# YiKwanwoo2/mycelium-fea-project

Measured on AMD Instinct MI355X. Metric: DOF solved/sec + CG iters to 1e-8; SpMV achieved HBM GB/s vs roofline, higher is better.
Workload: dtype f64 (CG; f32 AMG V-cycle); 1 GPU; C3_1M: 6x8 tiles, 1062000 DOF, 1008054 free DOF, 364342 elements, load step 20/40; n_dof=1062000, n_free_dof=1008054, n_elems=364342, precond=gamg, parallelism=1gpu, cg_kernel=lanes, n_lanes=353600

## Files before the change

mycelium-fea-project_amd/csrc/amg.hip:

```cpp
#include "amg_dev.hpp"

namespace mfea {

__device__ __forceinline__ int64_t setup_block(int x1, int64_t nmain = -1) {
  if (!x1) return nmain < 0 ? xcd_block() : xcd_block_n(nmain);
  return (blockIdx.x & 7) ? -1 : (int64_t)(blockIdx.x >> 3);
}


template <int ND>
__device__ __forceinline__ double dinv_row(const AmgLevD& L, int64_t i) {
  const AmgMatD& A = L.A;
  double g = 0.0;
  if (i - (threadIdx.x & 63) < A.rg.hi) {
    int64_t base;
    int w;
    slice_of(A, i, base, w);
    if (i >= A.rg.lo && i < A.rg.hi) {
      double D[ND * ND], Di[ND * ND];
      bload<ND>(A.val32, A.npos, base, D);
      binv<ND>(D, Di);
#pragma unroll
      for (int c = 0; c < ND * ND; ++c) L.dinv32[i * (ND * ND) + c] = (float)Di[c];
      double rs[ND];
// ... 1232 lines not shown
#pragma unroll
      for (int a = 0; a < 3; ++a) v.x[3 * row + a] = xk[a];
    } else {
      v.x[3 * row] = 0.0;
      v.x[3 * row + 1] = c == 3 ? 0.0 : (c == 2 ? dy_bot : dy_top);
      v.x[3 * row + 2] = 0.0;
    }
  }
  if (!block_publish<2>(acc, partials, ticket, red_out)) return;
  for (int64_t k = threadIdx.x; k < nzero; k += kBlock) zero[k] = 0.0;
  if (threadIdx.x == 0) cg_state_init(st, red_out[0], red_out[1], rtol, atol, norm, max_it, reg);
}

template <int BS, class F>
__device__ __forceinline__ void tile_rows(int64_t n, F&& f) {
  const int lane = threadIdx.x & 63;
  const int64_t nt = (n + 2 * BS - 1) / (2 * BS);
  for (int64_t tile = xcd_block(); tile < nt; tile += gridDim.x)
#pragma unroll
    for (int m = 0; m < 2; ++m) {
      const int64_t i = tile * (2 * BS) + m * BS + threadIdx.x;
      if (i - lane < n) f(i);
    }
}

template <int ND, bool FIRST, int BS, bool DIST, int KW = 1, bool TILE = false>
__global__ __launch_bounds__(BS) void k_amg_cg_w(int j, AmgLevD L0, AmgCg cg, Slot* slots, double* part,
                                                 AmgDist d) {
  double acc[4] = {0.0, 0.0, 0.0, 0.0};
  const int64_t stride = (int64_t)gridDim.x * BS;
  const int lane = threadIdx.x & 63;
  auto row = [&](int64_t i) {
    const int64_t ii = i < cg.hi ? i : cg.hi - 1;
    int64_t base;
    int w;
    slice_of(L0.A, ii, base, w);
    double y[ND], u[ND], r[ND];
    vload<ND>(cg.u, ii, u);
    vload<ND>(cg.r, ii, r);
#pragma unroll
    for (int a = 0; a < ND; ++a) y[a] = 0.0;
    sell_mac<ND, false, KW, true>(L0.A.col, L0.A.sym, L0.A.npos, base, w, cg.u, y);
    if (i < cg.lo || i >= cg.hi) return;
    if constexpr (DIST) {
      for (int t = d.gptr[i]; t < d.gptr[i + 1]; ++t) {
        const int64_t q = d.gslot[t];
        double s6[6], m[ND * ND], ug[ND];
#pragma unroll
        for (int c = 0; c < 6; ++c) s6[c] = d.sval[(int64_t)c * d.G + q];
        sym_to<ND>(s6, m);
        vload<ND>(d.urecv, d.grecv[t], ug);
#pragma unroll
        for (int a = 0; a < ND; ++a)
#pragma unroll
          for (int b = 0; b < ND; ++b) y[a] = fma(m[a * ND + b], ug[b], y[a]);
      }
    }
    vstore<ND>(cg.w, i, y);
#pragma unroll
    for (int a = 0; a < ND; ++a) {
      acc[0] = fma(r[a], u[a], acc[0]);
      acc[1] = fma(y[a], u[a], acc[1]);
      acc[2] = fma(r[a], r[a], acc[2]);
      acc[3] = fma(u[a], u[a], acc[3]);
    }
  };
  if constexpr (TILE) {
    tile_rows<BS>(cg.hi, row);
  } else {
    for (int64_t i = cg.lo64() + xcd_block() * BS + threadIdx.x; i - lane < cg.hi; i += stride) row(i);
  }
  store_block_partial<BS>(acc, part_buf(part, FIRST ? 0 : ((j & 1) ^ 1)));
  if (FIRST && blockIdx.x == 0 && threadIdx.x == 0) {
    Slot s0;
    s0.v[0] = s0.v[1] = s0.v[2] = s0.v[3] = 0.0;
    s0.alpha = s0.beta = s0.res = 0.0;
    s0.flag = kInit;
    s0.pad = 0;
    slots[0] = s0;
  }
}

template <int ND, int BS, int KW>
__global__ __launch_bounds__(BS) void k_amg_up_w(int j, int first, AmgLevD L, AmgLevD N, AmgCg cg, AmgFuseD f,
                                                 Slot* slots, double* part) {
  extern __shared__ float ul[];
  double acc[4] = {0.0, 0.0, 0.0, 0.0};
  const AmgMatD& T = L.PT;
  const int lane = threadIdx.x & 63;
  const int64_t n = cg.hi;
  const int64_t nt = (n + 2 * BS - 1) / (2 * BS);
  const float* src = N.coarsest ? N.x : N.e;
  for (int64_t tile = xcd_block(); tile < nt; tile += gridDim.x) {
    const int64_t r0 = tile * (2 * BS);
#pragma unroll
    for (int m = 0; m < 2; ++m) {
      const int64_t a = r0 + m * BS + threadIdx.x;
      if (a - lane >= n) continue;
      const int64_t aa = a < n ? a : n - 1;
      int64_t base;
      int w;
      slice_of(T, aa, base, w);
      const int64_t i = L.pt_row[aa];
      float y[ND];
      vload<ND>(L.t, i, y);
      sell_mac<ND, false, 3>(T.col, T.val32, T.npos, base, w, src, y);
      if (a < n) {
        vstore<ND>(cg.u, i, y);
        vstore<ND>(ul, i - r0, y);
      }
    }
    const int h0 = f.hptr[tile], h1 = f.hptr[tile + 1];
    for (int h = h0 + (int)threadIdx.x; h < h1; h += BS) {
      const int64_t a = f.hpt[h], i = f.hrow[h];
      const int sa = T.sptr[a >> 6], sb = T.sptr[(a >> 6) + 1];
      const int64_t base = (int64_t)sa * 64 + (a & 63);
      float y[ND];
      vload<ND>(L.t, i, y);
      sell_mac<ND, false, 3>(T.col, T.val32, T.npos, base, sb - sa, src, y);
      vstore<ND>(ul, 2 * BS + (h - h0), y);
    }
    __syncthreads();
#pragma unroll
    for (int m = 0; m < 2; ++m) {
      const int64_t i = r0 + m * BS + threadIdx.x;
      if (i - lane >= n) continue;
      const int64_t ii = i < n ? i : n - 1;
      int64_t base;
      int w;
      slice_of(L.A, ii, base, w);
      double y[ND], u[ND], r[ND];
      vload<ND>(ul, ii - r0, u);
      vload<ND>(cg.r, ii, r);
#pragma unroll
      for (int a = 0; a < ND; ++a) y[a] = 0.0;
      sell_mac<ND, false, KW, true>(f.lcol, L.A.sym, L.A.npos, base, w, (const float*)ul, y);
      if (i >= n) continue;
      vstore<ND>(cg.w, i, y);
#pragma unroll
      for (int a = 0; a < ND; ++a) {
        acc[0] = fma(r[a], u[a], acc[0]);
        acc[1] = fma(y[a], u[a], acc[1]);
        acc[2] = fma(r[a], r[a], acc[2]);
        acc[3] = fma(u[a], u[a], acc[3]);
      }
    }
    if (tile + gridDim.x < nt) __syncthreads();
  }
  store_block_partial<BS>(acc, part_buf(part, first ? 0 : ((j & 1) ^ 1)));
  if (first && blockIdx.x == 0 && threadIdx.x == 0) {
    Slot s0;
    s0.v[0] = s0.v[1] = s0.v[2] = s0.v[3] = 0.0;
    s0.alpha = s0.beta = s0.res = 0.0;
    s0.flag = kInit;
    s0.pad = 0;
    slots[0] = s0;
  }
}

struct PxLive {
  double alpha[kAmgPxSlots], beta[kAmgPxSlots];
  int64_t off[kAmgPxSlots];
  int n;
};
__device__ __forceinline__ void px_records(const Slot* __restrict__ slots, const AmgPx& px, PxLive& L) {
  if (threadIdx.x < 64) {
    const int t = threadIdx.x, k = px.k0 + t;
    bool run = false;
    double a = 0.0, b = 0.0;
    if (t < px.cnt) {
      const Slot& rec = slots[k + 1];
      run = rec.flag == kRun && rec.pad == 0;
      a = rec.alpha;
      b = rec.beta;
    }
    const unsigned long long m = __ballot(run);
    if (run) {
      const int q = __popcll(m & ((1ull << t) - 1ull));
      L.alpha[q] = a;
      L.beta[q] = b;
      L.off[q] = (int64_t)amg_px_slot(k) * px.stride;
    }
    if (t == 0) L.n = __popcll(m);
  }
  __syncthreads();
}
template <int ND>
__device__ __forceinline__ void px_row(const AmgCg& cg, const AmgPx& px, const PxLive& L, int64_t i) {
  const int n = L.n;
  if (n == 0) return;
  double p[ND], x[ND];
  vload<ND>(cg.p, i, p);
  vload<ND>(cg.x, i, x);
#pragma unroll 4
  for (int t = 0; t < n; ++t) {
    double u[ND];
    vload<ND>(px.uh + L.off[t], i, u);
    const double alpha = L.alpha[t], beta = L.beta[t];
#pragma unroll
    for (int a = 0; a < ND; ++a) {
      p[a] = fma(beta, p[a], u[a]);
      x[a] = fma(alpha, p[a], x[a]);
    }
  }
  vstore<ND>(cg.p, i, p);
  vstore<ND>(cg.x, i, x);
}
template <int ND>
__global__ __launch_bounds__(kCgBS) void k_amg_px_replay(AmgCg cg, const Slot* slots, AmgPx px) {
  __shared__ PxLive live;
  px_records(slots, px, live);
  const int64_t stride = (int64_t)gridDim.x * kCgBS;
  for (int64_t i = cg.lo + (int64_t)blockIdx.x * kCgBS + threadIdx.x; i < cg.hi; i += stride)
    px_row<ND>(cg, px, live, i);
}

template <int ND, int BS, bool REPLAY = false, bool TILE = false>
__global__ __launch_bounds__(BS) void k_amg_rnorm(AmgCg cg, double* cpart, const Slot* slots, AmgPx px) {
  __shared__ PxLive live;
  if constexpr (REPLAY) px_records(slots, px, live);
  double acc[4] = {0.0, 0.0, 0.0, 0.0};
  const int64_t stride = (int64_t)gridDim.x * BS;
  const int lane = threadIdx.x & 63;
  auto row = [&](int64_t i) {
    if (i < cg.lo || i >= cg.hi) return;
    double r[ND];
    vload<ND>(cg.r, i, r);
    if constexpr (REPLAY) px_row<ND>(cg, px, live, i);
#pragma unroll
    for (int a = 0; a < ND; ++a) acc[2] = fma(r[a], r[a], acc[2]);
  };
  if constexpr (TILE) {
// ... 523 lines not shown

void launch_amg_row0_inverse(hipStream_t s, const AmgCg& cg, int32_t* inv, int64_t n_rows) {
  (void)hipMemsetAsync(inv, 0xff, (size_t)n_rows * sizeof(int32_t), s);
  if (cg.hi <= cg.lo) return;
  hipLaunchKernelGGL(k_amg_row0_inverse, rows_grid(cg.hi - cg.lo), dim3(kBlock), 0, s, cg, inv);
}

void launch_amg_start(hipStream_t s, int nd, const SellOp& op, const uint8_t* code, double dy_top, double dy_bot,
                      const CgVecs& v, double* partials, unsigned* ticket, double* red_out, const AmgLevD& L0,
                      const AmgCg& cg, const int32_t* inv, double rtol, double atol, int norm, int max_it,
                      double reg, SolveState* st, double* zero, int64_t nzero, const BcForm& bc) {
  const dim3 grid((unsigned)grid_rows(op.N > 0 ? op.N : 1));
  with_bc(bc, [&](auto g, auto ld) {
    using GM = decltype(g);
    using LD = decltype(ld);
    if (nd == 2)
      hipLaunchKernelGGL((k_amg_start<2, GM, LD>), grid, dim3(kBlock), 0, s, op, code, dy_top, dy_bot, v, partials,
                         ticket, red_out, L0, cg, inv, rtol, atol, norm, max_it, reg, st, zero, nzero, g, ld);
    else
      hipLaunchKernelGGL((k_amg_start<3, GM, LD>), grid, dim3(kBlock), 0, s, op, code, dy_top, dy_bot, v, partials,
                         ticket, red_out, L0, cg, inv, rtol, atol, norm, max_it, reg, st, zero, nzero, g, ld);
  });
}

template <int ND, int BS>
static void w_bs(hipStream_t s, int j, bool first, const AmgLevD& L0, const AmgCg& cg, Slot* slots,
                 double* part, const AmgDist* d) {
  const dim3 g((unsigned)amg_w_grid(cg));
  const AmgDist dd = d ? *d : AmgDist{};
  if (d) {
    if (first) hipLaunchKernelGGL((k_amg_cg_w<ND, true, BS, true>), g, dim3(BS), 0, s, j, L0, cg, slots, part, dd);
    else hipLaunchKernelGGL((k_amg_cg_w<ND, false, BS, true>), g, dim3(BS), 0, s, j, L0, cg, slots, part, dd);
  } else if (cg.w_k == 2) {
    if (first) hipLaunchKernelGGL((k_amg_cg_w<ND, true, BS, false, 2>), g, dim3(BS), 0, s, j, L0, cg, slots, part, dd);
    else hipLaunchKernelGGL((k_amg_cg_w<ND, false, BS, false, 2>), g, dim3(BS), 0, s, j, L0, cg, slots, part, dd);
  } else {
    if (first) hipLaunchKernelGGL((k_amg_cg_w<ND, true, BS, false>), g, dim3(BS), 0, s, j, L0, cg, slots, part, dd);
    else hipLaunchKernelGGL((k_amg_cg_w<ND, false, BS, false>), g, dim3(BS), 0, s, j, L0, cg, slots, part, dd);
  }
}
template <int ND, int BS>
static void w_tile_bs(hipStream_t s, int j, bool first, const AmgLevD& L0, const AmgCg& cg, Slot* slots,
                      double* part) {
  const dim3 g((unsigned)amg_w_grid(cg));
  const AmgDist dd{};
  if (cg.w_k == 2) {
    if (first) hipLaunchKernelGGL((k_amg_cg_w<ND, true, BS, false, 2, true>), g, dim3(BS), 0, s, j, L0, cg, slots, part, dd);
    else hipLaunchKernelGGL((k_amg_cg_w<ND, false, BS, false, 2, true>), g, dim3(BS), 0, s, j, L0, cg, slots, part, dd);
  } else {
    if (first) hipLaunchKernelGGL((k_amg_cg_w<ND, true, BS, false, 1, true>), g, dim3(BS), 0, s, j, L0, cg, slots, part, dd);
    else hipLaunchKernelGGL((k_amg_cg_w<ND, false, BS, false, 1, true>), g, dim3(BS), 0, s, j, L0, cg, slots, part, dd);
  }
}
template <int ND>
static void w_nd(hipStream_t s, int j, bool first, const AmgLevD& L0, const AmgCg& cg, Slot* slots,
                 double* part, const AmgDist* d) {
  if (w_tiled(cg) && !d) {
    if (cg.w_tile == 1408) w_tile_bs<ND, 704>(s, j, first, L0, cg, slots, part);
    else w_tile_bs<ND, 512>(s, j, first, L0, cg, slots, part);
    return;
  }
  switch (amg_w_block(cg)) {
    case 512: w_bs<ND, 512>(s, j, first, L0, cg, slots, part, d); break;
    case 576: w_bs<ND, 576>(s, j, first, L0, cg, slots, part, d); break;
    case 640: w_bs<ND, 640>(s, j, first, L0, cg, slots, part, d); break;
    case 704: w_bs<ND, 704>(s, j, first, L0, cg, slots, part, d); break;
    case 768: w_bs<ND, 768>(s, j, first, L0, cg, slots, part, d); break;
    case 1024: w_bs<ND, 1024>(s, j, first, L0, cg, slots, part, d); break;
    default: w_bs<ND, kCgBS>(s, j, first, L0, cg, slots, part, d); break;
  }
}
void launch_amg_cg_w(hipStream_t s, int nd, int j, bool first, const AmgLevD& L0, const AmgCg& cg,
                     Slot* slots, double* part, const AmgDist* d) {
  if (nd == 2) w_nd<2>(s, j, first, L0, cg, slots, part, d);
  else w_nd<3>(s, j, first, L0, cg, slots, part, d);
}

template <int ND, int BS>
static void up_w_bs(hipStream_t s, int j, bool first, const AmgLevD& L0, const AmgLevD& L1, const AmgCg& cg,
                    const AmgFuseD& f, Slot* slots, double* part) {
  const dim3 g((unsigned)amg_w_grid(cg));
  const size_t lds = (size_t)(2 * BS + f.hcap) * ND * sizeof(float);
  const int fi = first ? 1 : 0;
  if (cg.w_k == 2) hipLaunchKernelGGL((k_amg_up_w<ND, BS, 2>), g, dim3(BS), lds, s, j, fi, L0, L1, cg, f, slots, part);
  else hipLaunchKernelGGL((k_amg_up_w<ND, BS, 1>), g, dim3(BS), lds, s, j, fi, L0, L1, cg, f, slots, part);
}
void launch_amg_up_w(hipStream_t s, int nd, int j, bool first, const AmgLevD& L0, const AmgLevD& L1,
                     const AmgCg& cg, const AmgFuseD& f, Slot* slots, double* part) {
  if (cg.w_tile == 1408) {
    if (nd == 2) up_w_bs<2, 704>(s, j, first, L0, L1, cg, f, slots, part);
    else up_w_bs<3, 704>(s, j, first, L0, L1, cg, f, slots, part);
  } else {
    if (nd == 2) up_w_bs<2, 512>(s, j, first, L0, L1, cg, f, slots, part);
    else up_w_bs<3, 512>(s, j, first, L0, L1, cg, f, slots, part);
  }
}

template <int ND, bool REPLAY>
static void rnorm_nd(hipStream_t s, const AmgCg& cg, double* cpart, const Slot* slots, const AmgPx& px) {
  const dim3 g((unsigned)amg_w_grid(cg));
  if (w_tiled(cg)) {
    if (cg.w_tile == 1408) hipLaunchKernelGGL((k_amg_rnorm<ND, 704, REPLAY, true>), g, dim3(704), 0, s, cg, cpart, slots, px);
    else hipLaunchKernelGGL((k_amg_rnorm<ND, 512, REPLAY, true>), g, dim3(512), 0, s, cg, cpart, slots, px);
    return;
  }
  switch (amg_w_block(cg)) {
    case 512: hipLaunchKernelGGL((k_amg_rnorm<ND, 512, REPLAY>), g, dim3(512), 0, s, cg, cpart, slots, px); break;
    case 576: hipLaunchKernelGGL((k_amg_rnorm<ND, 576, REPLAY>), g, dim3(576), 0, s, cg, cpart, slots, px); break;
    case 640: hipLaunchKernelGGL((k_amg_rnorm<ND, 640, REPLAY>), g, dim3(640), 0, s, cg, cpart, slots, px); break;
    case 704: hipLaunchKernelGGL((k_amg_rnorm<ND, 704, REPLAY>), g, dim3(704), 0, s, cg, cpart, slots, px); break;
    case 768: hipLaunchKernelGGL((k_amg_rnorm<ND, 768, REPLAY>), g, dim3(768), 0, s, cg, cpart, slots, px); break;
    case 1024: hipLaunchKernelGGL((k_amg_rnorm<ND, 1024, REPLAY>), g, dim3(1024), 0, s, cg, cpart, slots, px); break;
    default: hipLaunchKernelGGL((k_amg_rnorm<ND, kCgBS, REPLAY>), g, dim3(kCgBS), 0, s, cg, cpart, slots, px); break;
  }
}
void launch_amg_rnorm(hipStream_t s, int nd, const AmgCg& cg, double* cpart) {
  if (nd == 2) rnorm_nd<2, false>(s, cg, cpart, nullptr, AmgPx{});
  else rnorm_nd<3, false>(s, cg, cpart, nullptr, AmgPx{});
}
void launch_amg_rnorm_px(hipStream_t s, int nd, const AmgCg& cg, double* cpart, const Slot* slots,
                         const AmgPx& px) {
  if (nd == 2) rnorm_nd<2, true>(s, cg, cpart, slots, px);
  else rnorm_nd<3, true>(s, cg, cpart, slots, px);
}
void launch_amg_px_replay(hipStream_t s, int nd, const AmgCg& cg, const Slot* slots, const AmgPx& px) {
  if (cg.hi <= cg.lo) return;
  int64_t g = (cg.hi - cg.lo + kCgBS - 1) / kCgBS;
  g = g > kCgMaxG ? kCgMaxG : g;
  if (nd == 2) hipLaunchKernelGGL(k_amg_px_replay<2>, dim3((unsigned)g), dim3(kCgBS), 0, s, cg, slots, px);
  else hipLaunchKernelGGL(k_amg_px_replay<3>, dim3((unsigned)g), dim3(kCgBS), 0, s, cg, slots, px);
}

void launch_amg_gsum(hipStream_t s, const AmgCg& cg, const double* part_q, const AmgDist& d, int q) {
  double* all = d.gall[q];
  const int r = d.rank, zw = d.zero_w;
  switch (pu_of_grid(amg_w_grid(cg))) {
    case 1: hipLaunchKernelGGL(k_amg_gsum<1>, dim3(1), dim3(64), 0, s, part_q, all, r, zw, d.gsend); break;
    case 2: hipLaunchKernelGGL(k_amg_gsum<2>, dim3(1), dim3(64), 0, s, part_q, all, r, zw, d.gsend); break;
    case 4: hipLaunchKernelGGL(k_amg_gsum<4>, dim3(1), dim3(64), 0, s, part_q, all, r, zw, d.gsend); break;
    default: hipLaunchKernelGGL(k_amg_gsum<8>, dim3(1), dim3(64), 0, s, part_q, all, r, zw, d.gsend); break;
  }
}

void launch_amg_pack_u(hipStream_t s, int nd, const AmgCg& cg, const AmgDist& d) {
  if (d.n_send <= 0) return;
  if (nd == 2) hipLaunchKernelGGL(k_amg_pack_u<2>, rows_grid(d.n_send), dim3(kBlock), 0, s, cg, d);
  else hipLaunchKernelGGL(k_amg_pack_u<3>, rows_grid(d.n_send), dim3(kBlock), 0, s, cg, d);
}

template <int ND, int BS, bool DIST, bool LAZY = false>
static void upd_bs(hipStream_t s, int j, const AmgLevD& L0, const AmgCg& cg, Slot* slots,
                   SolveState* st, double* part, const AmgDist& d) {
  const int64_t gw = amg_w_grid(cg);
  int64_t gu = (cg.hi - cg.lo + BS - 1) / BS;
  gu = gu < 1 ? 1 : (gu > kCgMaxG ? kCgMaxG : gu);
  const dim3 g((unsigned)gu);
  switch (DIST ? 1 : pu_of_grid(gw)) {
    case 1: hipLaunchKernelGGL((k_amg_cg_update<ND, 1, BS, DIST, LAZY>), g, dim3(BS), 0, s, j, L0, cg, slots, st, part, d); break;
    case 2: hipLaunchKernelGGL((k_amg_cg_update<ND, 2, BS, DIST, LAZY>), g, dim3(BS), 0, s, j, L0, cg, slots, st, part, d); break;
    case 4: hipLaunchKernelGGL((k_amg_cg_update<ND, 4, BS, DIST, LAZY>), g, dim3(BS), 0, s, j, L0, cg, slots, st, part, d); break;
    default: hipLaunchKernelGGL((k_amg_cg_update<ND, 8, BS, DIST, LAZY>), g, dim3(BS), 0, s, j, L0, cg, slots, st, part, d); break;
  }
}
template <int ND>
static void upd_nd(hipStream_t s, int j, const AmgLevD& L0, const AmgCg& cg, Slot* slots,
                   SolveState* st, double* part, const AmgDist* d, bool lazy) {
  if (d) upd_bs<ND, kCgBS, true>(s, j, L0, cg, slots, st, part, *d);
  else if (lazy) upd_bs<ND, kCgBS, false, true>(s, j, L0, cg, slots, st, part, AmgDist{});
// ... 114 lines not shown
```

mycelium-fea-project_amd/csrc/amg_dev.hpp:

```cpp
#pragma once
#include "amg_kernels.hpp"
#include "device_util.hpp"

namespace mfea {

template <int ND, class T, class C>
__device__ __forceinline__ void bload(const T* __restrict__ v, int64_t , int64_t q, C* m) {
#pragma unroll
  for (int c = 0; c < ND * ND; ++c) m[c] = (C)v[q * (ND * ND) + c];
}
template <int ND, class T, class C>
__device__ __forceinline__ void bstore(T* __restrict__ v, int64_t , int64_t q, const C* m) {
#pragma unroll
  for (int c = 0; c < ND * ND; ++c) v[q * (ND * ND) + c] = (T)m[c];
}
template <int ND>
constexpr int nsym() { return ND * (ND + 1) / 2; }
template <int ND, class T, class C>
__device__ __forceinline__ void bload_sym(const T* __restrict__ v, int64_t , int64_t q, C* m) {
  constexpr int NS = nsym<ND>();
  C t[NS];
#pragma unroll
  for (int c = 0; c < NS; ++c) t[c] = (C)v[q * NS + c];
  if constexpr (ND == 2) {
// ... 133 lines not shown
  return slot_wave(M, t0, t1, q, row, k, xcd_block());
}

__device__ __forceinline__ int32_t uniform_load(const int32_t* p, int64_t i) {
  return ((const __attribute__((address_space(4))) int32_t*)p)[i];
}
__device__ __forceinline__ void slice_of(const AmgMatD& M, int64_t row, int64_t& base, int& width) {
  const int s = __builtin_amdgcn_readfirstlane((int)(row >> 6));
  const int a = uniform_load(M.sptr, s), b = uniform_load(M.sptr, s + 1);
  base = (int64_t)a * 64 + (row & 63);
  width = b - a;
}

template <int ND>
constexpr int mac_unroll() { return ND == 2 ? 4 : 2; }

template <int ND, int U, int S, bool SUB, bool SYM, class TV, class XP, class C, class CI>
__device__ __forceinline__ void sell_step(const CI* __restrict__ col, const TV* __restrict__ val,
                                          int64_t base, int k, int ws, int sub, XP x, C* y) {
  int32_t c[U];
  int64_t q[U];
  C m[U][ND * ND], xc[U][ND];
#pragma unroll
  for (int u = 0; u < U; ++u) {
    q[u] = k + u < ws ? base + (int64_t)((k + u) * S + sub) * 64 : base;
    c[u] = k + u < ws ? col[q[u]] : -1;
  }
#pragma unroll
  for (int u = 0; u < U; ++u) {
    if constexpr (SYM) bload_sym<ND>(val, 0, q[u], m[u]);
    else bload<ND>(val, 0, q[u], m[u]);
  }
#pragma unroll
  for (int u = 0; u < U; ++u) vload<ND>(x, c[u] >= 0 ? c[u] : 0, xc[u]);
#pragma unroll
  for (int u = 0; u < U; ++u) {
#pragma unroll
    for (int b = 0; b < ND; ++b) {
      if constexpr (SYM) xc[u][b] = keep_or_zero(xc[u][b], c[u] >= 0);
      else xc[u][b] = c[u] >= 0 ? xc[u][b] : (C)0;
    }
#pragma unroll
    for (int a = 0; a < ND; ++a)
#pragma unroll
      for (int b = 0; b < ND; ++b)
        y[a] = fma(SUB ? -m[u][a * ND + b] : m[u][a * ND + b], xc[u][b], y[a]);
  }
}
template <int ND, int UMAX, int S, bool SUB, bool SYM, class TV, class XP, class C, class CI>
__device__ __forceinline__ int sell_step_by(const CI* __restrict__ col, const TV* __restrict__ val,
                                            int64_t base, int k, int rem, int ws, int sub, XP x, C* y) {
  if (UMAX >= 16 && rem > 8) {
    sell_step<ND, (UMAX >= 16 ? 16 : 1), S, SUB, SYM>(col, val, base, k, ws, sub, x, y);
    return 16;
  }
  if (UMAX >= 8 && rem > 4) {
    sell_step<ND, (UMAX >= 8 ? 8 : 1), S, SUB, SYM>(col, val, base, k, ws, sub, x, y);
    return 8;
  }
  if (UMAX >= 4 && rem > 2) {
    sell_step<ND, (UMAX >= 4 ? 4 : 1), S, SUB, SYM>(col, val, base, k, ws, sub, x, y);
    return 4;
  }
  if (rem > 1) {
    sell_step<ND, 2, S, SUB, SYM>(col, val, base, k, ws, sub, x, y);
    return 2;
  }
  sell_step<ND, 1, S, SUB, SYM>(col, val, base, k, ws, sub, x, y);
  return 1;
}
template <int ND, int UMAX, int S, bool SUB, bool SYM, class TV, class XP, class C, class CI>
__device__ __forceinline__ void sell_steps(const CI* __restrict__ col, const TV* __restrict__ val,
                                           int64_t base, int wu, int ws, int sub, XP x, C* y) {
  for (int k = 0; k < wu;) k += sell_step_by<ND, UMAX, S, SUB, SYM>(col, val, base, k, wu - k, ws, sub, x, y);
}
template <int ND, bool SUB, int K = 2, bool SYM = false, class TV, class XP, class C, class CI>
__device__ __forceinline__ void sell_mac(const CI* __restrict__ col, const TV* __restrict__ val,
                                         int64_t , int64_t base, int w,
                                         XP x, C* y) {
  constexpr int UMAX = mac_unroll<ND>() << (K - 1);
  sell_steps<ND, UMAX, 1, SUB, SYM>(col, val, base, w, w, 0, x, y);
}

template <int ND, class TD, class C>
__device__ __forceinline__ void dinv_load(const TD* __restrict__ dinv, int64_t i, C* Di) {
#pragma unroll
  for (int c = 0; c < ND * ND; ++c) Di[c] = (C)dinv[i * (ND * ND) + c];
}
template <int ND, class C>
__device__ __forceinline__ void dinv_mul(const C* Di, C s, const C* v, C* o) {
#pragma unroll
  for (int a = 0; a < ND; ++a) {
    C acc = 0;
#pragma unroll
    for (int b = 0; b < ND; ++b) acc = fma(Di[a * ND + b], v[b], acc);
    o[a] = s * acc;
  }
}
template <int ND, class TD, class C>
__device__ __forceinline__ void dinv_apply(const TD* __restrict__ dinv, int64_t , int64_t i, C s,
                                           const C* v, C* o) {
  C Di[ND * ND];
  dinv_load<ND>(dinv, i, Di);
  dinv_mul<ND>(Di, s, v, o);
}

template <int ND, bool TX, int U, class TX_, class TY_>
__device__ __forceinline__ void pair_sum_u(int t0, int t1, const int32_t* __restrict__ la,
                                           const int32_t* __restrict__ lb, const TX_* __restrict__ X,
                                           const TY_* __restrict__ Y, double* C) {
  for (int t = t0; t < t1; t += U) {
    int32_t ia[U], ib[U];
#pragma unroll
    for (int u = 0; u < U; ++u) {
      const int tt = t + u < t1 ? t + u : t0;
      ia[u] = la[tt];
      ib[u] = lb[tt];
    }
    double x[U][ND * ND], y[U][ND * ND];
#pragma unroll
    for (int u = 0; u < U; ++u) {
      bload<ND>(X, 0, ia[u], x[u]);
      bload<ND>(Y, 0, ib[u], y[u]);
    }
#pragma unroll
    for (int u = 0; u < U; ++u) {
#pragma unroll
      for (int c = 0; c < ND * ND; ++c) x[u][c] = keep_or_zero(x[u][c], t + u < t1);
      if (TX) mtm_acc<ND>(x[u], y[u], C);
      else mm_acc<ND>(x[u], y[u], C);
    }
  }
}
template <int ND, bool TX, class TX_, class TY_>
__device__ __forceinline__ void pair_sum(int t0, int t1, const int32_t* __restrict__ la,
                                         const int32_t* __restrict__ lb, const TX_* __restrict__ X,
                                         int64_t , const TY_* __restrict__ Y, int64_t , double* C) {
  pair_sum_u<ND, TX, 4>(t0, t1, la, lb, X, Y, C);
}
template <int ND, int U, class TX_>
__device__ __forceinline__ void list_sum_u(int t0, int t1, const int32_t* __restrict__ la,
                                           const TX_* __restrict__ X, double* S) {
  for (int t = t0; t < t1; t += U) {
    int32_t ia[U];
#pragma unroll
    for (int u = 0; u < U; ++u) ia[u] = la[t + u < t1 ? t + u : t0];
    double x[U][ND * ND];
#pragma unroll
    for (int u = 0; u < U; ++u) bload<ND>(X, 0, ia[u], x[u]);
#pragma unroll
    for (int u = 0; u < U; ++u)
#pragma unroll
      for (int c = 0; c < ND * ND; ++c) S[c] += keep_or_zero(x[u][c], t + u < t1);
  }
}
template <int ND, class TX_>
__device__ __forceinline__ void list_sum(int t0, int t1, const int32_t* __restrict__ la,
                                         const TX_* __restrict__ X, int64_t , double* S) {
  list_sum_u<ND, 4>(t0, t1, la, X, S);
}

constexpr double kRhoFloor = 2.0;
constexpr double kRhoSafety = 1.45;

__device__ __forceinline__ double amg_omega(const double* __restrict__ om) {
  return (4.0 / 3.0) / (om[0] > 0.0 ? om[0] : fmax(kRhoFloor, om[1] / kRhoSafety));
// ... 22 lines not shown
```

mycelium-fea-project_amd/csrc/amg_kernels.hpp:

```cpp
#pragma once
#include <hip/hip_runtime.h>
#include <stdint.h>

#include "kernels.hpp"

namespace mfea {

struct RowRange {
  int64_t lo = 0, hi = 0;
  int64_t p0 = 0, p1 = 0;
  int64_t pf = 0, pl = 0;
  int64_t s0 = 0, s1 = 0;
  int64_t rows() const { return hi > lo ? hi - lo : 0; }
  __host__ __device__ int64_t lo64() const { return lo & ~(int64_t)63; }
  int64_t span() const { return hi > lo ? hi - lo64() : 0; }
  int64_t npos() const { return p1 > p0 ? p1 - p0 : 0; }
};

struct AmgMatD {
  int64_t n = 0;
  int64_t npos = 0;
  int32_t wmax = 0;
  RowRange rg;
  const int32_t* sptr = nullptr;
// ... 125 lines not shown
  float* dt = nullptr;
  float* lov = nullptr;
  float* upv = nullptr;
  double* y = nullptr;
};
void launch_sweep_setup(hipStream_t s, int nd, const SweepD& sw, const AmgLevD& L0);
void launch_sweep(hipStream_t s, int nd, const SweepD& sw, const AmgCg& cg, const int32_t* gate);

struct AmgDist {
  int rank = 0;
  int zero_w = 0;
  double* gall[2] = {nullptr, nullptr};
  double* gsend = nullptr;
  const int32_t* gptr = nullptr;
  const int32_t* gslot = nullptr;
  const int32_t* grecv = nullptr;
  const double* sval = nullptr;
  int64_t G = 0;
  const int32_t* send_rows = nullptr;
  int64_t n_send = 0;
  double* usend = nullptr;
  const double* urecv = nullptr;
};

void launch_amg_a0(hipStream_t s, int nd, const AmgLevD& L0, const SellOp& sop, const int32_t* row0,
                   const int32_t* a0_ptr, const int32_t* a0_a, double reg, bool full = false);
constexpr int kSetupDinv = 1, kSetupP = 2, kSetupAP = 4, kSetupAC = 8, kSetupAll = 15;
void launch_amg_level_setup(hipStream_t s, int nd, const AmgLevD& L, const AmgLevD* next, bool level0,
                            int stage = kSetupAll);
void launch_amg_compact_setup(hipStream_t s, int nd, const AmgLevD* lev, int nlev, int coll = 0, int l0 = 0);
constexpr int kCompactPT = 1, kCompactRT = 2, kCompactAT = 4, kCompactAll = 7;
void launch_amg_compact_level(hipStream_t s, int nd, const AmgLevD* lev, int l, int parts);
void launch_amg_down(hipStream_t s, int nd, const AmgLevD& L, const AmgLevD& N);
void launch_amg_up(hipStream_t s, int nd, const AmgLevD& L, const AmgLevD& N, float* e);
bool launch_amg_setup_fused(hipStream_t s, int nd, const AmgLevD* lev, int nlev, int coll,
                            const AmgMergeD* mg = nullptr);
void launch_amg_vcycle(hipStream_t s, int nd, const AmgLevD* lev, int nlev, const AmgCg& cg,
                       int tail, const int32_t* gate, int l0 = 0, const AmgMergeD* mg = nullptr);
constexpr int kStepResid = 0, kStepRestrict = 1, kStepProlong = 2, kStepPost = 3;
void launch_amg_vstep(hipStream_t s, int nd, const AmgLevD* lev, int l, const AmgCg& cg, int step,
                      const int32_t* gate);
void launch_xpack(hipStream_t s, const void* src, const int32_t* idx, int64_t n, int width, int bytes, void* buf);
constexpr int kMaxXPairs = 48;
struct XPairs {
  int n = 0;
  int64_t off[kMaxXPairs + 1] = {};
  const void* src[kMaxXPairs] = {};
  void* dst[kMaxXPairs] = {};
  const int32_t* sidx[kMaxXPairs] = {};
  const int32_t* ridx[kMaxXPairs] = {};
};
void launch_xcopy(hipStream_t s, const XPairs& pr, int width, int bytes);
struct GallCopy {
  int n = 0;
  const double* gsend[64] = {};
  double* gall[64] = {};
  int rank[64] = {};
};
void launch_gall_copy(hipStream_t s, const GallCopy& g);
void launch_xunpack(hipStream_t s, const void* buf, const int32_t* idx, int64_t n, int width, int bytes, void* dst);
void launch_amg_xinit_rows(hipStream_t s, int nd, const AmgLevD& N, const int32_t* rows, int64_t n,
                           const int32_t* gate);
void launch_amg_bound_max(hipStream_t s, double* const* omegas, int n);
int amg_restrict_lanes(const AmgLevD& L);
int amg_op_lanes(const AmgLevD& L);
int amg_down_lanes(const AmgLevD& L);
int amg_up_lanes(const AmgLevD& L);
bool amg_compact_ok(const AmgLevD* lev, int nlev, int l0);
int amg_tail_level(const int64_t* rows, int nlev, int64_t max_rows);
void launch_amg_cg_init(hipStream_t s, int nd, const AmgLevD& L0, const AmgCg& cg, const double* b_row);
void launch_amg_cg_w(hipStream_t s, int nd, int j, bool first, const AmgLevD& L0, const AmgCg& cg,
                     Slot* slots, double* part, const AmgDist* d = nullptr);
struct AmgFuseD {
  int on = 0;
  int hcap = 0;
  const int32_t* hptr = nullptr;
  const int32_t* hrow = nullptr;
  const int32_t* hpt = nullptr;
  const int16_t* lcol = nullptr;
};
constexpr int64_t kAmgFuseLds = 48 * 1024;
inline bool amg_fuse_tile_ok(int64_t B) { return B == 1408 || B == 1024; }
inline int64_t amg_fuse_halo_cap(int nd, int64_t B) { return kAmgFuseLds / (4 * nd) - B; }
void launch_amg_up_w(hipStream_t s, int nd, int j, bool first, const AmgLevD& L0, const AmgLevD& L1,
                     const AmgCg& cg, const AmgFuseD& f, Slot* slots, double* part);
void launch_amg_row0_inverse(hipStream_t s, const AmgCg& cg, int32_t* inv, int64_t n_rows);
void launch_amg_start(hipStream_t s, int nd, const SellOp& op, const uint8_t* code, double dy_top, double dy_bot,
                      const CgVecs& v, double* partials, unsigned* ticket, double* red_out, const AmgLevD& L0,
                      const AmgCg& cg, const int32_t* inv, double rtol, double atol, int norm, int max_it,
                      double reg, SolveState* st, double* zero, int64_t nzero, const BcForm& bc);
void launch_amg_rnorm(hipStream_t s, int nd, const AmgCg& cg, double* cpart);
constexpr int kAmgPxSlots = 17;
struct AmgPx {
  const float* uh = nullptr;
  int64_t stride = 0;
  int k0 = 0;
  int cnt = 0;
};
__host__ __device__ inline int amg_px_slot(int k) { return k == 0 ? 0 : 1 + (k - 1) % (kAmgPxSlots - 1); }
void launch_amg_rnorm_px(hipStream_t s, int nd, const AmgCg& cg, double* cpart, const Slot* slots,
                         const AmgPx& px);
void launch_amg_px_replay(hipStream_t s, int nd, const AmgCg& cg, const Slot* slots, const AmgPx& px);
void launch_amg_gsum(hipStream_t s, const AmgCg& cg, const double* part_q, const AmgDist& d, int q);
void launch_amg_pack_u(hipStream_t s, int nd, const AmgCg& cg, const AmgDist& d);
void launch_amg_cg_update(hipStream_t s, int nd, int j, const AmgLevD& L0, const AmgCg& cg,
                          Slot* slots, SolveState* st, double* part,
                          const AmgDist* d = nullptr, bool lazy = false);
void launch_amg_finish(hipStream_t s, int nd, const AmgCg& cg, double* x_row);
int64_t amg_w_grid(const AmgCg& cg);

}
```

mycelium-fea-project_amd/csrc/device_util.hpp:

```cpp
#pragma once
#include <type_traits>

#include "kernels.hpp"

namespace mfea {

__device__ __forceinline__ double wave_sum(double v) {
#pragma unroll
  for (int off = 32; off > 0; off >>= 1) v += __shfl_xor(v, off, 64);
  return v;
}

template <int CTRL>
__device__ __forceinline__ double dpp_d(double v) {
  const int lo = __builtin_amdgcn_update_dpp(0, __double2loint(v), CTRL, 0xF, 0xF, false);
  const int hi = __builtin_amdgcn_update_dpp(0, __double2hiint(v), CTRL, 0xF, 0xF, false);
  return __hiloint2double(hi, lo);
}
__device__ __forceinline__ double readlane_d(double v, int lane) {
  const int lo = __builtin_amdgcn_readlane(__double2loint(v), lane);
  const int hi = __builtin_amdgcn_readlane(__double2hiint(v), lane);
  return __hiloint2double(hi, lo);
}
__device__ __forceinline__ double wave_allsum(double v) {
// ... 332 lines not shown
#pragma unroll
    for (int u = 0; u < U; ++u) {
      idx[u] = base + (int64_t)(k0 + u < len ? k0 + u : k0) * 64;
      j[u] = k0 + u < len ? op.s_col[idx[u]] : 0;
    }
    uint8_t c[U];
#pragma unroll
    for (int u = 0; u < U; ++u) c[u] = k0 + u < len && j[u] >= op.nf ? code[j[u]] : 3;
#pragma unroll
    for (int u = 0; u < U; ++u) {
      if (c[u] != 3) {
        const double dy = c[u] == 2 ? dy_bot : dy_top;
        kx = fma(op.val[1 * G + idx[u]], dy, kx);
        ky = fma(op.val[3 * G + idx[u]], dy, ky);
        kz = fma(op.val[4 * G + idx[u]], dy, kz);
      }
    }
  }
  const double k3[3] = {kx, ky, kz};
  load_rhs(ld, lr, dy_top, k3, b);
}

__device__ __forceinline__ void cg_state_init(SolveState* st, double bb, double zz, double rtol, double atol,
                                              int norm, int max_it, double reg) {
  const double ref = norm == 1 ? zz : bb;
  const double t = rtol * rtol * ref, a2 = atol * atol;
  st->tol2 = t > a2 ? t : a2;
  st->rtol2 = rtol * rtol;
  st->atol2 = a2;
  st->reg = reg;
  st->bb0 = bb;
  st->res0 = ref;
  st->res_final = ref;
  st->base = 0;
  st->max_it = max_it;
  st->norm = norm;
  st->done = 0;
  st->iters = 0;
  st->status = 0;
  st->closed = 0;
}

constexpr int kCgBS = 256;
constexpr int kCgMaxG = kCgMaxPartials;

__device__ __forceinline__ void block_mac(const double V[6], const double u[3], double y[3]) {
  y[0] = fma(V[0], u[0], fma(V[1], u[1], fma(V[2], u[2], y[0])));
  y[1] = fma(V[1], u[0], fma(V[3], u[1], fma(V[4], u[2], y[1])));
  y[2] = fma(V[2], u[0], fma(V[4], u[1], fma(V[5], u[2], y[2])));
}

template <bool BLOCK>
__device__ __forceinline__ void apply_m(const double* M, const double r[3], double u[3]) {
  if (BLOCK) {
    sym_apply(M, r, u);
  } else {
#pragma unroll
    for (int a = 0; a < 3; ++a) u[a] = M[a] * r[a];
  }
}

__device__ __forceinline__ double* part_buf(double* part, int par) {
  return part + (size_t)par * 4 * kCgMaxG;
}

template <int PU>
__device__ __forceinline__ void wave_partials(const double* __restrict__ p, double s[4]) {
  const int lane = threadIdx.x & 63;
  double t[PU][4];
#pragma unroll
  for (int k = 0; k < PU; ++k) {
#pragma unroll
    for (int c = 0; c < 4; ++c) t[k][c] = p[c * kCgMaxG + lane + 64 * k];
  }
#pragma unroll
  for (int c = 0; c < 4; ++c) {
    double a = 0.0;
#pragma unroll
    for (int k = 0; k < PU; ++k) a += t[k][c];
    s[c] = wave_allsum(a);
  }
}

template <int BS = kCgBS>
__device__ __forceinline__ void store_block_partial(double (&acc)[4], double* __restrict__ p) {
  constexpr int NW = BS / 64;
  __shared__ double lds[NW * 4];
  const int lane = threadIdx.x & 63, wid = threadIdx.x >> 6;
#pragma unroll
  for (int c = 0; c < 4; ++c) acc[c] = wave_allsum(acc[c]);
  if (lane == 0) {
#pragma unroll
    for (int c = 0; c < 4; ++c) lds[wid * 4 + c] = acc[c];
  }
  if (NW > 1) asm volatile("s_waitcnt lgkmcnt(0)\n\ts_barrier" ::: "memory");
  else asm volatile("s_waitcnt lgkmcnt(0)" ::: "memory");
  if (threadIdx.x == 0) {
#pragma unroll
    for (int c = 0; c < 4; ++c) {
      double s = lds[c];
      for (int w = 1; w < NW; ++w) s += lds[w * 4 + c];
      p[c * kCgMaxG + blockIdx.x] = s;
    }
  }
}

struct CgScalars {
  double alpha, beta, res;
  int status;
};
__device__ __forceinline__ CgScalars cg_scalars(const double S[4], int f0, double g0, double a0,
                                                double tol2, int it, int max_it, int norm) {
  CgScalars c;
  c.res = norm == 1 ? S[3] : S[2];
  const bool first = f0 == kInit;
  c.beta = first ? 0.0 : S[0] / g0;
  const double den = first ? S[1] : S[1] - c.beta * S[0] / a0;
  c.alpha = S[0] / den;
  if (f0 != kRun && f0 != kInit) c.status = kStop;
  else if (!(c.res > tol2)) c.status = isfinite(c.res) ? kConverged : kBreakdown;
  else if (it >= max_it) c.status = kMaxit;
  else c.status = ((den > 0.0) && isfinite(c.alpha) && isfinite(c.beta)) ? kRun : kBreakdown;
  return c;
}

__device__ __forceinline__ double cg_close_sum(const double* __restrict__ cpart, int G) {
  const int lane = threadIdx.x & 63;
  double a = 0.0;
#pragma unroll
  for (int k = 0; k < kCgMaxG / 64; ++k) {
    const int b = lane + 64 * k;
    a += b < G ? cpart[2 * kCgMaxG + b] : 0.0;
  }
  return wave_allsum(a);
}
__device__ __forceinline__ bool cg_close_converged(double rr, double tol2) {
  return !(rr > tol2) && isfinite(rr);
}

__device__ __forceinline__ void cg_record(Slot* slots, int j, const double S[4],
                                          const CgScalars& c) {
  if (blockIdx.x == 0 && threadIdx.x == 0) {
    Slot sl;
    sl.v[0] = S[0]; sl.v[1] = S[1]; sl.v[2] = S[2]; sl.v[3] = S[3];
    sl.alpha = c.alpha;
    sl.beta = c.beta;
    sl.res = c.res;
    sl.flag = c.status;
    sl.pad = 0;
    slots[j + 1] = sl;
  }
}

template <bool TRACE, int BS = kCgBS>
__device__ __forceinline__ void trace_point(unsigned long long* trace, int point, double dep) {
  if (TRACE) {
    unsigned long long t;
    asm volatile("s_memrealtime %0\n\ts_waitcnt lgkmcnt(0)" : "=s"(t) : "v"(dep));
    if ((threadIdx.x & 63) == 0)
      trace[((size_t)blockIdx.x * (BS / 64) + (threadIdx.x >> 6)) * 4 + point] = t;
  }
}

}
```

Baseline: 1.057 billion DOF/s.

## Add dedicated halo wave and prefetch first SpMV row loads before barrier in up_w

The fused prolongation+W SpMV kernel gets an extra 64-thread wave that computes the halo prolongation rows. The main waves now run only their owned rows. Before the block barrier, the main waves also issue the first slice's column and symmetric-value loads and the residual load for the m=0 row, so those global loads overlap the barrier wait. The cost is higher register pressure from the prefetched SellFirst state, an extra wave per block, and a single wave for the halo, which may become the critical path when halos are large.

Result: slower. 1.020 billion DOF/s (-3.5%).

```diff
diff --git a/mycelium-fea-project_amd/csrc/amg.hip b/mycelium-fea-project_amd/csrc/amg.hip
--- a/mycelium-fea-project_amd/csrc/amg.hip
+++ b/mycelium-fea-project_amd/csrc/amg.hip
@@ -1338,72 +1338,105 @@
 }
 
 template <int ND, int BS, int KW>
-__global__ __launch_bounds__(BS) void k_amg_up_w(int j, int first, AmgLevD L, AmgLevD N, AmgCg cg, AmgFuseD f,
-                                                 Slot* slots, double* part) {
+__global__ __launch_bounds__(BS + (kAmgUpWHaloWave ? 64 : 0)) void k_amg_up_w(int j, int first, AmgLevD L, AmgLevD N,
+                                                                            AmgCg cg, AmgFuseD f, Slot* slots,
+                                                                            double* part) {
   extern __shared__ float ul[];
+  constexpr int UMAX = mac_unroll<ND>() << (KW - 1);
   double acc[4] = {0.0, 0.0, 0.0, 0.0};
   const AmgMatD& T = L.PT;
-  const int lane = threadIdx.x & 63;
+  const bool own = !kAmgUpWHaloWave || __builtin_amdgcn_readfirstlane((int)threadIdx.x) < BS;
   const int64_t n = cg.hi;
   const int64_t nt = (n + 2 * BS - 1) / (2 * BS);
   const float* src = N.coarsest ? N.x : N.e;
   for (int64_t tile = xcd_block(); tile < nt; tile += gridDim.x) {
     const int64_t r0 = tile * (2 * BS);
-#pragma unroll
-    for (int m = 0; m < 2; ++m) {
-      const int64_t a = r0 + m * BS + threadIdx.x;
-      if (a - lane >= n) continue;
-      const int64_t aa = a < n ? a : n - 1;
-      int64_t base;
-      int w;
-      slice_of(T, aa, base, w);
-      const int64_t i = L.pt_row[aa];
-      float y[ND];
-      vload<ND>(L.t, i, y);
-      sell_mac<ND, false, 3>(T.col, T.val32, T.npos, base, w, src, y);
-      if (a < n) {
-        vstore<ND>(cg.u, i, y);
-        vstore<ND>(ul, i - r0, y);
+    const int tid = threadIdx.x, lane = tid & 63;
+    auto halo = [&](int t, int step) {
+      const int h0 = f.hptr[tile], h1 = f.hptr[tile + 1];
+      for (int h = h0 + t; h < h1; h += step) {
+        const int64_t a = f.hpt[h], i = f.hrow[h];
+        const int sa = T.sptr[a >> 6], sb = T.sptr[(a >> 6) + 1];
+        const int64_t base = (int64_t)sa * 64 + (a & 63);
+        float y[ND];
+        vload<ND>(L.t, i, y);
+        sell_mac<ND, false, 3>(T.col, T.val32, T.npos, base, sb - sa, src, y);
+        vstore<ND>(ul, 2 * BS + (h - h0), y);
       }
-    }
-    const int h0 = f.hptr[tile], h1 = f.hptr[tile + 1];
-    for (int h = h0 + (int)threadIdx.x; h < h1; h += BS) {
-      const int64_t a = f.hpt[h], i = f.hrow[h];
-      const int sa = T.sptr[a >> 6], sb = T.sptr[(a >> 6) + 1];
-      const int64_t base = (int64_t)sa * 64 + (a & 63);
-      float y[ND];
-      vload<ND>(L.t, i, y);
-      sell_mac<ND, false, 3>(T.col, T.val32, T.npos, base, sb - sa, src, y);
-      vstore<ND>(ul, 2 * BS + (h - h0), y);
-    }
-    __syncthreads();
-#pragma unroll
-    for (int m = 0; m < 2; ++m) {
-      const int64_t i = r0 + m * BS + threadIdx.x;
-      if (i - lane >= n) continue;
-      const int64_t ii = i < n ? i : n - 1;
-      int64_t base;
-      int w;
-      slice_of(L.A, ii, base, w);
-      double y[ND], u[ND], r[ND];
-      vload<ND>(ul, ii - r0, u);
-      vload<ND>(cg.r, ii, r);
-#pragma unroll
-      for (int a = 0; a < ND; ++a) y[a] = 0.0;
-      sell_mac<ND, false, KW, true>(f.lcol, L.A.sym, L.A.npos, base, w, (const float*)ul, y);
-      if (i >= n) continue;
-      vstore<ND>(cg.w, i, y);
-#pragma unroll
-      for (int a = 0; a < ND; ++a) {
-        acc[0] = fma(r[a], u[a], acc[0]);
-        acc[1] = fma(y[a], u[a], acc[1]);
-        acc[2] = fma(r[a], r[a], acc[2]);
-        acc[3] = fma(u[a], u[a], acc[3]);
+    };
+    SellFirst<ND, UMAX, int16_t> fs;
+    int64_t fbase = 0;
+    int fw = 0;
+    double fr[ND];
+    if (own) {
+#pragma unroll
+      for (int m = 0; m < 2; ++m) {
+        const int64_t a = r0 + m * BS + tid;
+        if (a - lane >= n) continue;
+        const int64_t aa = a < n ? a : n - 1;
+        int64_t base;
+        int w;
+        slice_of(T, aa, base, w);
+        const int64_t i = L.pt_row[aa];
+        float y[ND];
+        vload<ND>(L.t, i, y);
+        sell_mac<ND, false, 3>(T.col, T.val32, T.npos, base, w, src, y);
+        if (a < n) {
+          vstore<ND>(cg.u, i, y);
+          vstore<ND>(ul, i - r0, y);
+        }
       }
+      if constexpr (!kAmgUpWHaloWave) halo(tid, BS);
+      if constexpr (kAmgUpWEarlyLoads) {
+        const int64_t i = r0 + tid;
+        const int64_t ii = i < n ? i : n - 1;
+        slice_of(L.A, ii, fbase, fw);
+        vload<ND>(cg.r, ii, fr);
+        sell_first_issue<ND>(f.lcol, L.A.sym, fbase, fw, fs);
+      }
+    } else {
+      halo(lane, 64);
+    }
+    if constexpr (kAmgUpWEarlyLoads) asm volatile("s_waitcnt lgkmcnt(0)\n\ts_barrier" ::: "memory");
+    else __syncthreads();
+    if (own) {
+#pragma unroll
+      for (int m = 0; m < 2; ++m) {
+        const int64_t i = r0 + m * BS + tid;
+        if (i - lane >= n) continue;
+        const int64_t ii = i < n ? i : n - 1;
+        const bool early = kAmgUpWEarlyLoads && m == 0;
+        int64_t base;
+        int w;
+        double y[ND], u[ND], r[ND];
+        if (early) {
+          base = fbase;
+          w = __builtin_amdgcn_readfirstlane(fw);
+#pragma unroll
+          for (int a = 0; a < ND; ++a) r[a] = fr[a];
+        } else {
+          slice_of(L.A, ii, base, w);
+        }
+        vload<ND>(ul, ii - r0, u);
+        if (!early) vload<ND>(cg.r, ii, r);
+#pragma unroll
+        for (int a = 0; a < ND; ++a) y[a] = 0.0;
+        if (early) sell_first_rest<ND>(fs, f.lcol, L.A.sym, base, w, (const float*)ul, y);
+        else sell_mac<ND, false, KW, true>(f.lcol, L.A.sym, L.A.npos, base, w, (const float*)ul, y);
+        if (i >= n) continue;
+        vstore<ND>(cg.w, i, y);
+#pragma unroll
+        for (int a = 0; a < ND; ++a) {
+          acc[0] = fma(r[a], u[a], acc[0]);
+          acc[1] = fma(y[a], u[a], acc[1]);
+          acc[2] = fma(r[a], r[a], acc[2]);
+          acc[3] = fma(u[a], u[a], acc[3]);
+        }
+      }
     }
     if (tile + gridDim.x < nt) __syncthreads();
   }
-  store_block_partial<BS>(acc, part_buf(part, first ? 0 : ((j & 1) ^ 1)));
+  store_block_partial<BS, (kAmgUpWHaloWave ? 1 : 0)>(acc, part_buf(part, first ? 0 : ((j & 1) ^ 1)));
   if (first && blockIdx.x == 0 && threadIdx.x == 0) {
     Slot s0;
     s0.v[0] = s0.v[1] = s0.v[2] = s0.v[3] = 0.0;
@@ -2093,8 +2126,9 @@
   const dim3 g((unsigned)amg_w_grid(cg));
   const size_t lds = (size_t)(2 * BS + f.hcap) * ND * sizeof(float);
   const int fi = first ? 1 : 0;
-  if (cg.w_k == 2) hipLaunchKernelGGL((k_amg_up_w<ND, BS, 2>), g, dim3(BS), lds, s, j, fi, L0, L1, cg, f, slots, part);
-  else hipLaunchKernelGGL((k_amg_up_w<ND, BS, 1>), g, dim3(BS), lds, s, j, fi, L0, L1, cg, f, slots, part);
+  const dim3 b(BS + (kAmgUpWHaloWave ? 64 : 0));
+  if (cg.w_k == 2) hipLaunchKernelGGL((k_amg_up_w<ND, BS, 2>), g, b, lds, s, j, fi, L0, L1, cg, f, slots, part);
+  else hipLaunchKernelGGL((k_amg_up_w<ND, BS, 1>), g, b, lds, s, j, fi, L0, L1, cg, f, slots, part);
 }
 void launch_amg_up_w(hipStream_t s, int nd, int j, bool first, const AmgLevD& L0, const AmgLevD& L1,
                      const AmgCg& cg, const AmgFuseD& f, Slot* slots, double* part) {
diff --git a/mycelium-fea-project_amd/csrc/amg_dev.hpp b/mycelium-fea-project_amd/csrc/amg_dev.hpp
--- a/mycelium-fea-project_amd/csrc/amg_dev.hpp
+++ b/mycelium-fea-project_amd/csrc/amg_dev.hpp
@@ -239,6 +239,99 @@
   sell_steps<ND, UMAX, 1, SUB, SYM>(col, val, base, w, w, 0, x, y);
 }
 
+template <int ND, int UMAX, class CI>
+struct SellFirst {
+  CI c[UMAX];
+  double t[UMAX][nsym<ND>()];
+  int u;
+};
+template <int ND>
+constexpr int sell_first_early() { return mac_unroll<ND>(); }
+template <int UMAX>
+__device__ __forceinline__ int sell_first_width(int w) {
+  static_assert(UMAX <= 8, "sell_step_by's widths up to 8");
+  if (w <= 0) return 0;
+  if (UMAX >= 8 && w > 4) return 8;
+  if (UMAX >= 4 && w > 2) return 4;
+  return w > 1 ? 2 : 1;
+}
+template <int ND, int A, int B, int UMAX, class CI>
+__device__ __forceinline__ void sell_first_load(bool on, const CI* __restrict__ col,
+                                                const double* __restrict__ val, int64_t base, int w,
+                                                SellFirst<ND, UMAX, CI>& s) {
+  constexpr int NS = nsym<ND>();
+  if (on) {
+    int64_t q[B - A];
+#pragma unroll
+    for (int u = A; u < B; ++u) {
+      q[u - A] = u < w ? base + (int64_t)u * 64 : base;
+      s.c[u] = u < w ? col[q[u - A]] : (CI)-1;
+    }
+#pragma unroll
+    for (int u = A; u < B; ++u)
+#pragma unroll
+      for (int c = 0; c < NS; ++c) s.t[u][c] = val[q[u - A] * NS + c];
+  } else {
+#pragma unroll
+    for (int u = A; u < B; ++u) {
+      s.c[u] = (CI)-1;
+#pragma unroll
+      for (int c = 0; c < NS; ++c) s.t[u][c] = 0.0;
+    }
+  }
+}
+template <int ND, int UMAX, class CI>
+__device__ __forceinline__ void sell_first_issue(const CI* __restrict__ col, const double* __restrict__ val,
+                                                 int64_t base, int w, SellFirst<ND, UMAX, CI>& s) {
+  constexpr int E = sell_first_early<ND>();
+  s.u = sell_first_width<UMAX>(w);
+  sell_first_load<ND, 0, 1>(s.u > 0, col, val, base, w, s);
+  sell_first_load<ND, 1, 2>(s.u > 1, col, val, base, w, s);
+  if constexpr (UMAX >= 4 && E >= 4) sell_first_load<ND, 2, 4>(s.u > 2, col, val, base, w, s);
+  if constexpr (UMAX >= 8 && E >= 8) sell_first_load<ND, 4, 8>(s.u > 4, col, val, base, w, s);
+}
+template <int ND, int A, int B, int UMAX, class CI, class XP>
+__device__ __forceinline__ void sell_first_gather(const SellFirst<ND, UMAX, CI>& s, XP x, double (&xc)[UMAX][ND]) {
+#pragma unroll
+  for (int u = A; u < B; ++u) vload<ND>(x, s.c[u] >= 0 ? s.c[u] : 0, xc[u]);
+}
+template <int ND, int A, int B, int UMAX, class CI>
+__device__ __forceinline__ void sell_first_fma(const SellFirst<ND, UMAX, CI>& s, double (&xc)[UMAX][ND], double* y) {
+#pragma unroll
+  for (int u = A; u < B; ++u) {
+    double m[ND * ND];
+    bload_sym<ND>(s.t[u], 0, 0, m);
+#pragma unroll
+    for (int b = 0; b < ND; ++b) xc[u][b] = keep_or_zero(xc[u][b], s.c[u] >= 0);
+#pragma unroll
+    for (int a = 0; a < ND; ++a)
+#pragma unroll
+      for (int b = 0; b < ND; ++b) y[a] = fma(m[a * ND + b], xc[u][b], y[a]);
+  }
+}
+template <int ND, int UMAX, class CI, class XP>
+__device__ __forceinline__ void sell_first_rest(SellFirst<ND, UMAX, CI>& s, const CI* __restrict__ col,
+                                                const double* __restrict__ val, int64_t base, int w, XP x,
+                                                double* y) {
+  const int su = __builtin_amdgcn_readfirstlane(s.u);
+  if constexpr (UMAX >= 4 && sell_first_early<ND>() < 4) sell_first_load<ND, 2, 4>(su > 2, col, val, base, w, s);
+  if constexpr (UMAX >= 8 && sell_first_early<ND>() < 8) sell_first_load<ND, 4, 8>(su > 4, col, val, base, w, s);
+  double xc[UMAX][ND];
+  if (su > 0) sell_first_gather<ND, 0, 1>(s, x, xc);
+  if (su > 1) sell_first_gather<ND, 1, 2>(s, x, xc);
+  if constexpr (UMAX >= 4)
+    if (su > 2) sell_first_gather<ND, 2, 4>(s, x, xc);
+  if constexpr (UMAX >= 8)
+    if (su > 4) sell_first_gather<ND, 4, 8>(s, x, xc);
+  if (su > 0) sell_first_fma<ND, 0, 1>(s, xc, y);
+  if (su > 1) sell_first_fma<ND, 1, 2>(s, xc, y);
+  if constexpr (UMAX >= 4)
+    if (su > 2) sell_first_fma<ND, 2, 4>(s, xc, y);
+  if constexpr (UMAX >= 8)
+    if (su > 4) sell_first_fma<ND, 4, 8>(s, xc, y);
+  for (int k = su; k < w;) k += sell_step_by<ND, UMAX, 1, false, true>(col, val, base, k, w - k, w, 0, x, y);
+}
+
 template <int ND, class TD, class C>
 __device__ __forceinline__ void dinv_load(const TD* __restrict__ dinv, int64_t i, C* Di) {
 #pragma unroll
diff --git a/mycelium-fea-project_amd/csrc/amg_kernels.hpp b/mycelium-fea-project_amd/csrc/amg_kernels.hpp
--- a/mycelium-fea-project_amd/csrc/amg_kernels.hpp
+++ b/mycelium-fea-project_amd/csrc/amg_kernels.hpp
@@ -231,6 +231,8 @@
 constexpr int64_t kAmgFuseLds = 48 * 1024;
 inline bool amg_fuse_tile_ok(int64_t B) { return B == 1408 || B == 1024; }
 inline int64_t amg_fuse_halo_cap(int nd, int64_t B) { return kAmgFuseLds / (4 * nd) - B; }
+constexpr bool kAmgUpWHaloWave = true;
+constexpr bool kAmgUpWEarlyLoads = true;
 void launch_amg_up_w(hipStream_t s, int nd, int j, bool first, const AmgLevD& L0, const AmgLevD& L1,
                      const AmgCg& cg, const AmgFuseD& f, Slot* slots, double* part);
 void launch_amg_row0_inverse(hipStream_t s, const AmgCg& cg, int32_t* inv, int64_t n_rows);
diff --git a/mycelium-fea-project_amd/csrc/device_util.hpp b/mycelium-fea-project_amd/csrc/device_util.hpp
--- a/mycelium-fea-project_amd/csrc/device_util.hpp
+++ b/mycelium-fea-project_amd/csrc/device_util.hpp
@@ -438,18 +438,18 @@
   }
 }
 
-template <int BS = kCgBS>
+template <int BS = kCgBS, int XW = 0>
 __device__ __forceinline__ void store_block_partial(double (&acc)[4], double* __restrict__ p) {
   constexpr int NW = BS / 64;
   __shared__ double lds[NW * 4];
   const int lane = threadIdx.x & 63, wid = threadIdx.x >> 6;
 #pragma unroll
   for (int c = 0; c < 4; ++c) acc[c] = wave_allsum(acc[c]);
-  if (lane == 0) {
+  if (lane == 0 && (XW == 0 || wid < NW)) {
 #pragma unroll
     for (int c = 0; c < 4; ++c) lds[wid * 4 + c] = acc[c];
   }
-  if (NW > 1) asm volatile("s_waitcnt lgkmcnt(0)\n\ts_barrier" ::: "memory");
+  if (NW + XW > 1) asm volatile("s_waitcnt lgkmcnt(0)\n\ts_barrier" ::: "memory");
   else asm volatile("s_waitcnt lgkmcnt(0)" ::: "memory");
   if (threadIdx.x == 0) {
 #pragma unroll
```
